# 111116/zdr

Measured on AMD Instinct MI355X. Metric: Msamples/s fwd+PRB-bwd, cbox 512x512 spp=256, higher is better.
Workload: dtype f32; 1 GPU; cbox path integrator 512x512 spp=256, forward + PRB backward w.r.t. the 1024x1024x4 material (BASELINE configs[2]); sampler=cmj, accel=brute, rccl_ranks=1, backend=none

## Files before the change

include/zdr.h:

```cpp
#ifndef ZDR_H
#define ZDR_H
#include <stdint.h>

#ifdef __cplusplus
extern "C" {
#endif

#define ZDR_VERSION_STRING "zdr-mi355x 0.3 (gfx950)"
#define ZDR_ABI_VERSION 4

enum { ZDR_OK = 0, ZDR_E_INVALID = -1, ZDR_E_HIP = -2, ZDR_E_UNSUPPORTED = -3, ZDR_E_NOMEM = -4 };

enum { ZDR_COLLOCATED = 0, ZDR_DIRECT = 1, ZDR_PATH = 2, ZDR_UVGRAD = 3 };
enum { ZDR_SAMPLER_CMJ = 0, ZDR_SAMPLER_PMJ02BN = 1 };
enum { ZDR_ACCEL_AUTO = 0, ZDR_ACCEL_BRUTE = 1, ZDR_ACCEL_BVH = 2 };
enum { ZDR_PRB_EXPECTATION = 0, ZDR_PRB_DETACHED = 1, ZDR_PRB_LITERAL = 2 };
#define ZDR_MAX_MATERIALS 16

typedef struct zdr_scene zdr_scene;

typedef struct {
    float fov;
    float origin[3], target[3], up[3];
} zdr_camera;
// ... 71 lines not shown
int zdr_render_stats(zdr_scene *scene, const zdr_render_params *params, const float *material,
                     uint64_t counters[8], void *stream);

int zdr_scene_check(zdr_scene *scene, void *stream);

int zdr_trace_closest(zdr_scene *scene, const float *rays, uint32_t n, int32_t *inst_prim, float *bary_t, void *stream);
int zdr_trace_any(zdr_scene *scene, const float *rays, uint32_t n, int32_t *occluded, void *stream);

int zdr_sampler_dump(zdr_scene *scene, int32_t sampler, uint32_t seed, uint32_t spp, const int32_t *queries,
                     uint32_t n, int32_t nvert, int32_t rr_depth, float *out, void *stream);

int zdr_vertex_sampler_dump(zdr_scene *scene, int32_t integrator, int32_t sampler, uint32_t seed, uint32_t spp,
                            const int32_t *queries, uint32_t n, int32_t nvert, int32_t rr_depth, float *out,
                            int32_t *batched, void *stream);

int zdr_path_dump(zdr_scene *scene, const zdr_render_params *params, const float *material, const float *d_image,
                  const int32_t *queries, uint32_t n, int32_t maxv, float *out, void *stream);

int zdr_debug_build_accel(const float *tri_xyz, uint32_t ntris, int accel, float *nodes_out, uint32_t nodes_cap,
                          uint32_t *nnodes, uint32_t *stack_entries, int32_t *order_out, float *isect_out);

int zdr_debug_never_occluders(const float *tri_xyz, uint32_t ntris, const uint8_t *is_light_tri, uint8_t *never_out);

#ifdef __cplusplus
}
#endif
#endif
```

zdr_amd/_native.py:

```python
from __future__ import annotations

import ctypes as C
import os

HERE = os.path.dirname(os.path.abspath(__file__))
LIB_PATH = os.path.join(HERE, "csrc", "libzdr_hip.so")

COLLOCATED, DIRECT, PATH, UVGRAD = 0, 1, 2, 3
SAMPLER_CMJ, SAMPLER_PMJ02BN = 0, 1
ACCEL_AUTO, ACCEL_BRUTE, ACCEL_BVH = 0, 1, 2
ABI_VERSION = 4
MAX_MATERIALS = 16
PRB_MODES = {"expectation": 0, "detached": 1, "literal": 2}
INTEGRATORS = {"collocated": COLLOCATED, "direct": DIRECT, "path": PATH}
SAMPLERS = {"cmj": SAMPLER_CMJ, "corrmj": SAMPLER_CMJ, "pmj02bn": SAMPLER_PMJ02BN}
ACCELS = {"auto": ACCEL_AUTO, "brute": ACCEL_BRUTE, "bvh": ACCEL_BVH}
COUNTER_NAMES = ("samples", "closest_rays", "closest_hits", "shadow_rays", "shaded_vertices",
                 "emitter_hits_bsdf", "nan_samples", "shadow_rays_traced")

EXPORTS = ("zdr_version", "zdr_abi_version", "zdr_last_error", "zdr_scene_create", "zdr_scene_destroy", "zdr_scene_info",
           "zdr_scene_set_emissions", "zdr_scene_set_envmap", "zdr_scene_set_pmj02bn_tables", "zdr_render_forward", "zdr_render_backward",
           "zdr_render_stats", "zdr_scene_check", "zdr_trace_closest", "zdr_trace_any", "zdr_sampler_dump", "zdr_vertex_sampler_dump", "zdr_path_dump", "zdr_debug_build_accel", "zdr_debug_never_occluders",
           "zdr_scene_set_material_slots", "zdr_render_forward_materials", "zdr_render_backward_materials",
           "zdr_scene_set_envmap_texture", "zdr_render_backward_env", "zdr_render_backward_materials_env",
           "zdr_scene_set_emission_values", "zdr_render_backward_emission", "zdr_render_backward_materials_emission")


class CameraPOD(C.Structure):
    _fields_ = [("fov", C.c_float), ("origin", C.c_float * 3), ("target", C.c_float * 3), ("up", C.c_float * 3)]


class RenderParams(C.Structure):
    _fields_ = [
        ("struct_size", C.c_uint32), ("integrator", C.c_int32), ("sampler", C.c_int32), ("width", C.c_int32), ("height", C.c_int32),
        ("spp", C.c_uint32), ("seed", C.c_uint32), ("use_tent", C.c_int32),
        ("x0", C.c_int32), ("y0", C.c_int32), ("x1", C.c_int32), ("y1", C.c_int32),
        ("sample_begin", C.c_uint32), ("sample_end", C.c_uint32),
        ("max_depth", C.c_int32), ("rr_depth", C.c_int32),
        ("camera", CameraPOD), ("tex_h", C.c_int32), ("tex_w", C.c_int32),
        ("tile_shard_index", C.c_int32), ("tile_shard_count", C.c_int32), ("prb_mode", C.c_int32),
    ]


class SceneInfo(C.Structure):
    _fields_ = [("ntris", C.c_uint32), ("nverts", C.c_uint32), ("ninst", C.c_uint32), ("light_count", C.c_uint32),
# ... 27 lines not shown
    L.zdr_scene_set_emissions.argtypes = [vp, fp, vp]
    L.zdr_scene_set_envmap.argtypes = [vp, fp, C.c_uint32, C.c_uint32, fp, ip, fp, C.c_uint32, C.c_uint32]
    L.zdr_scene_set_pmj02bn_tables.argtypes = [vp, vp, C.c_uint32, C.c_uint32, vp, C.c_uint32, C.c_uint32]
    L.zdr_render_forward.argtypes = [vp, C.POINTER(RenderParams), fp, fp, vp]
    L.zdr_render_backward.argtypes = [vp, C.POINTER(RenderParams), fp, fp, fp, vp]
    L.zdr_scene_set_material_slots.argtypes = [vp, ip, vp]
    L.zdr_render_forward_materials.argtypes = [vp, C.POINTER(RenderParams), fp, ip, C.c_uint32, fp, vp]
    L.zdr_render_backward_materials.argtypes = [vp, C.POINTER(RenderParams), fp, fp, ip, C.c_uint32, fp, vp]
    L.zdr_scene_set_envmap_texture.argtypes = [vp, fp, vp]
    L.zdr_render_backward_env.argtypes = [vp, C.POINTER(RenderParams), fp, fp, fp, fp, vp]
    L.zdr_render_backward_materials_env.argtypes = [vp, C.POINTER(RenderParams), fp, fp, ip, C.c_uint32, fp, fp, vp]
    L.zdr_scene_set_emission_values.argtypes = [vp, fp, vp]
    L.zdr_render_backward_emission.argtypes = [vp, C.POINTER(RenderParams), fp, fp, fp, fp, vp]
    L.zdr_render_backward_materials_emission.argtypes = [vp, C.POINTER(RenderParams), fp, fp, ip, C.c_uint32, fp, fp, vp]
    L.zdr_render_stats.argtypes = [vp, C.POINTER(RenderParams), fp, C.POINTER(C.c_uint64), vp]
    L.zdr_scene_check.argtypes = [vp, vp]
    L.zdr_trace_closest.argtypes = [vp, fp, C.c_uint32, ip, fp, vp]
    L.zdr_trace_any.argtypes = [vp, fp, C.c_uint32, ip, vp]
    L.zdr_sampler_dump.argtypes = [vp, C.c_int32, C.c_uint32, C.c_uint32, ip, C.c_uint32, C.c_int32, C.c_int32, fp, vp]
    L.zdr_vertex_sampler_dump.argtypes = [vp, C.c_int32, C.c_int32, C.c_uint32, C.c_uint32, ip, C.c_uint32, C.c_int32, C.c_int32, fp, C.POINTER(C.c_int32), vp]
    L.zdr_path_dump.argtypes = [vp, C.POINTER(RenderParams), fp, fp, ip, C.c_uint32, C.c_int32, fp, vp]
    L.zdr_debug_build_accel.argtypes = [fp, C.c_uint32, C.c_int, fp, C.c_uint32, C.POINTER(C.c_uint32), C.POINTER(C.c_uint32), ip, fp]
    L.zdr_debug_never_occluders.argtypes = [fp, C.c_uint32, vp, vp]
    for name in EXPORTS:
        getattr(L, name)
    if L.zdr_abi_version() != ABI_VERSION:
        raise ZdrError(f"{LIB_PATH} speaks ABI {L.zdr_abi_version()}, this binding ABI {ABI_VERSION}: rebuild (python -m zdr_amd.build --force)")
    _LIB = L
    return L


def check(rc: int):
    if rc != 0:
        raise ZdrError(f"libzdr_hip error {rc}: {lib().zdr_last_error().decode()}")
```

zdr_amd/csrc/accel.h:

```cpp
#pragma once
#include "scene.h"

#ifndef ZDR_MIN_WAVES
#define ZDR_MIN_WAVES 4
#endif
#ifndef ZDR_MIN_WAVES_ENV
#define ZDR_MIN_WAVES_ENV 4
#endif
#ifndef ZDR_MIN_WAVES_BVH
#define ZDR_MIN_WAVES_BVH 5
#endif
#ifndef ZDR_MIN_WAVES_BWD
#define ZDR_MIN_WAVES_BWD 4
#endif
#ifndef ZDR_POOL_SLOTS
#define ZDR_POOL_SLOTS 103
#endif
#ifndef ZDR_POOL_SLOTS_BVH
#define ZDR_POOL_SLOTS_BVH 56
#endif
#ifndef ZDR_MIN_WAVES_BWD_BVH
#define ZDR_MIN_WAVES_BWD_BVH 4
#endif

// ... 2 lines not shown
typedef const v4f __attribute__((address_space(4))) *const_v4f_ptr;
ZD const_v4f_ptr as_constant(const float4 *p) { return (const_v4f_ptr)(uintptr_t)p; }
ZD float4 f4(v4f a) { return make_float4(a.x, a.y, a.z, a.w); }

ZD bool tri_test(float4 N, float4 U, float4 V, f3 o, f3 d, float tmin, float tmax, float &t) {
    float nd = fmaf(N.z, d.z, fmaf(N.y, d.y, N.x * d.x));
    float no = fmaf(N.z, o.z, fmaf(N.y, o.y, N.x * o.x));
    float tt = (N.w - no) * rcp(nd);
    float px = fmaf(d.x, tt, o.x), py = fmaf(d.y, tt, o.y), pz = fmaf(d.z, tt, o.z);
    float uu = fmaf(U.z, pz, fmaf(U.y, py, U.x * px)) + U.w;
    float vv = fmaf(V.z, pz, fmaf(V.y, py, V.x * px)) + V.w;
    float c = fminf(fminf(uu, vv), 1.0f - (uu + vv));
    t = tt;
    return (tt > tmin) & (tt < tmax) & (c >= 0.0f);
}

ZD void hit_barycentrics(const DScene &S, Hit &h, f3 o, f3 d) {
    if (h.slot < 0) return;
    float4 U = S.isect[3 * (size_t)h.slot + 1], V = S.isect[3 * (size_t)h.slot + 2];
    f3 p = o + d * h.t;
    h.u = U.x * p.x + U.y * p.y + U.z * p.z + U.w;
    h.v = V.x * p.x + V.y * p.y + V.z * p.z + V.w;
}

typedef float v2f __attribute__((ext_vector_type(2)));
ZD v2f splat(float a) { v2f r = {a, a}; return r; }
ZD v2f pfma(v2f a, v2f b, v2f c) { return __builtin_elementwise_fma(a, b, c); }

struct PairHit { v2f t, c; };
ZD PairHit pair_test(const_v4f_ptr q, f3 o, f3 d) {
    v4f q0 = q[0], q1 = q[1];
    v2f dx = splat(d.x), dy = splat(d.y), dz = splat(d.z), ox = splat(o.x), oy = splat(o.y), oz = splat(o.z);
    v2f nd = pfma(q1.xy, dz, pfma(q0.zw, dy, q0.xy * dx));
    v2f no = pfma(q1.xy, oz, pfma(q0.zw, oy, q0.xy * ox));
    v2f tn = q1.zw - no;
    v2f r = {rcp(nd.x), rcp(nd.y)};
    PairHit h;
    h.t = tn * r;
    v2f px = pfma(dx, h.t, ox), py = pfma(dy, h.t, oy), pz = pfma(dz, h.t, oz);
    v2f e[4];
#pragma unroll
    for (int k = 0; k < 4; k++) {
        v4f a = q[2 + 2 * k], b = q[3 + 2 * k];
        e[k] = pfma(b.xy, pz, pfma(a.zw, py, a.xy * px)) + b.zw;
    }
    h.c.x = fminf(fminf(fminf(e[0].x, e[1].x), e[2].x), e[3].x);
    h.c.y = fminf(fminf(fminf(e[0].y, e[1].y), e[2].y), e[3].y);
    return h;
}

// ... 350 lines not shown
```

zdr_amd/csrc/integrators.h:

```cpp
#pragma once
#include <type_traits>
#include "accel.h"
#include "internal.h"
#include "microfacet.h"
#include "zdr.h"

ZD float tent_warp1(float u) {
    return (u < 0.5f) ? (fsqrt(2.0f * u) - 1.0f) : (1.0f - fsqrt(2.0f - 2.0f * u));
}

template <int SK, bool PACKED = false>
ZD void pixel_ray(const RenderCfg &R, const SamplerCfg &C, Sampler &smp, int x, int y, f3 &o, f3 &d) {
    f2 off = PACKED ? sampler_pixel_offset<SK>(C, smp) : sampler_next2<SK>(C, smp);
    if (R.use_tent) { off.x = tent_warp1(off.x) + 0.5f; off.y = tent_warp1(off.y) + 0.5f; }
    float px = R.two_over_w * ((float)x + off.x) - 1.0f;
    float py = R.two_over_h * ((float)y + off.y) - 1.0f;
    py *= R.aspect;
    px *= R.cam_tan; py *= R.cam_tan;
    o = ld3(R.cam_o);
    d = normalize((ld3(R.cam_right) * px - ld3(R.cam_upp) * py) + ld3(R.cam_fwd));
}

struct Counters { uint32_t c[8]; };
enum { C_SAMPLES, C_CLOSEST, C_HITS, C_SHADOW, C_SHADED, C_EMIT_BSDF, C_NAN, C_SHADOW_TRACED };
// ... 249 lines not shown
    else m = read_bsdf(io.material, it.uv, R.tex_h, R.tex_w);
    x.diffuse = mk3(m.x, m.y, m.z); x.roughness = m.w;
    COUNT(C_SHADED);
    if (BWD) {
        pv.uv = it.uv; pv.bW = mk3(0.0f); pv.cL = 0.0f; pv.dfLdr = 0.0f; pv.bpq = mk3(0.0f); pv.c = 0.0f; pv.dfdr = 0.0f;
        pv.T = mk3(0.0f); pv.fLW = mk3(0.0f); pv.bnorm = mk3(0.0f); pv.neeM = mk3(0.0f); pv.dlnp = 0.0f; pv.rr = 0;
    }
    x.onb = make_onb(it.ns);
    x.wo = to_local(x.onb, -ps.d);
    x.pre = (SK == 0) && !ENV && cmj_can_batch(C);
    x.u_lobe = 0.0f; x.u_dir.x = 0.0f; x.u_dir.y = 0.0f; x.i_rr = 0u;
    if (x.pre) {
        const VertexSamples v = cmj_vertex_samples(C, ps.smp);
        x.u_lobe = v.u_lobe; x.u_dir = v.u_dir; x.i_rr = v.i_rr;
        x.light = sample_light<ENV, LG>(S, it.p, v.u_pick, [&]() { return v.u_prim; }, [&]() { return v.u_pt; }, env_uv, mesh_light);
    } else {
        float u_pick = sampler_next<SK>(C, ps.smp);
        x.light = sample_light<ENV, LG>(S, it.p, u_pick, [&]() { return sampler_next<SK>(C, ps.smp); }, [&]() { return sampler_next2<SK>(C, ps.smp); }, env_uv, mesh_light);
    }
    x.wil = to_local(x.onb, x.light.wi);
    return x;
}

template <bool BWD, bool EG = false>
ZD NeeTerms nee_terms(const ShadeCtx &x, f3 beta_in, f3 *env_w = nullptr) {
    NeeTerms n; n.dL = n.bW = n.fLW = n.neeM = mk3(0.0f); n.cL = 0.0f; n.dfLdr = 0.0f;
    GgxTerms g = ggx_terms(x.wo, x.wil, x.roughness);
    f3 bsdf = ggx_brdf_from(g, x.wil, x.diffuse);
    float pb = ggx_pdf_from(g, x.wo, x.wil);
    float mis = balanced_heuristic(x.light.pdf, pb);
    float inv_dn = rcp(fmaxf(x.light.pdf, 1e-4f));
    n.dL = (((beta_in * bsdf) * mis) * x.light.eval) * inv_dn;
    if constexpr (EG) *env_w = ((beta_in * bsdf) * mis) * inv_dn;
    if (BWD) {
        f3 W = (x.light.eval * mis) * inv_dn;
        float dlnpL;
        n.bW = beta_in * W; n.cL = x.wil.z * ZDR_INV_PI; n.dfLdr = ggx_dfdr_from(g, x.wo, x.wil, x.roughness, dlnpL);
        n.fLW = bsdf * W;
        float pbf = (x.light.pdf + pb > 1e-4f) ? pb * rcp(x.light.pdf + pb) : 0.0f;
        n.neeM = ((beta_in * bsdf) * W) * (pbf * dlnpL);
    }
    return n;
}
template <bool BWD>
ZD void nee_apply(PathState &ps, PathVertex &pv, const NeeTerms &n) {
    ps.L = ps.L + n.dL;
    if (BWD) { pv.bW = n.bW; pv.cL = n.cL; pv.dfLdr = n.dfLdr; pv.fLW = n.fLW; pv.neeM = n.neeM; }
}

template <int SK, bool BWD>
ZD bool sample_bsdf(const RenderCfg &R, const SamplerCfg &C, const ShadeCtx &x, PathState &ps, const Interaction &it, PathVertex &pv) {
    float u_lobe = x.u_lobe; f2 u_dir = x.u_dir;
    if (!x.pre) { u_lobe = sampler_next<SK>(C, ps.smp); u_dir = sampler_next2<SK>(C, ps.smp); }
    f3 wi_local = ggx_sample(x.wo, x.roughness, u_lobe, u_dir);
    GgxTerms g = ggx_terms(x.wo, wi_local, x.roughness);
    ps.pdf_bsdf = ggx_pdf_from(g, x.wo, wi_local);
    f3 wi = to_world(x.onb, wi_local);
    bool stop = (dot(wi, it.ng) < 1e-4f) || (wi_local.z < 1e-4f);
    const f3 beta_in = ps.beta;
    float q = 1.0f;
    int rr_kind = 0;
    if (!stop) {
        ps.o = offset_ray_origin(it.p, it.ng); ps.d = wi;
        f3 f = ggx_brdf_from(g, wi_local, x.diffuse);
        float inv_p = rcp(ps.pdf_bsdf);
        ps.beta = ps.beta * (f * inv_p);
        if (ps.depth >= R.rr_depth) {
            float l = 0.212671f * ps.beta.x + 0.715160f * ps.beta.y + 0.072169f * ps.beta.z;
            if (l == 0.0f) stop = true;
            else {
                q = fmaxf(l, 0.05f);
                float r = x.pre ? cmj_next_with_index(C, ps.smp, x.i_rr) : sampler_next<SK>(C, ps.smp);
                if (r >= q) stop = true;
                else { ps.beta = ps.beta * rcp(q); rr_kind = (l >= 1.0f) ? 2 : ((l >= 0.05f) ? 1 : 0); }
            }
        }
        if (BWD && !stop) {
            float inv_pq = inv_p * rcp(q);
            pv.bpq = beta_in * inv_pq; pv.c = wi_local.z * ZDR_INV_PI; pv.dfdr = ggx_dfdr_from(g, x.wo, wi_local, x.roughness, pv.dlnp);
            pv.T = f * inv_pq;
            pv.rr = rr_kind;
            if (rr_kind == 2) pv.bnorm = ps.beta;
            if (R.prb_mode == ZDR_PRB_LITERAL) pv.bnorm = beta_in * (f * inv_p);
        }
    }
    ps.depth++;
    if (ps.depth >= R.max_depth) stop = true;
    return stop;
}

struct VertexRays { bool shadow, stop; f3 sd; float stmax; };
template <int SK, bool BWD, bool STATS, bool ENV, bool MT = false, bool EG = false, bool LG = false>
ZD VertexRays path_vertex_begin(const DScene &S, const RenderCfg &R, const SamplerCfg &C, const KernelIO &io,
                                PathState &ps, const Interaction &it, PathVertex &pv, NeeTerms &n, Counters &cnt, EnvTerm *env = nullptr, EmitTerm *emit = nullptr) {
    f2 env_uv; env_uv.x = -1.0f; env_uv.y = 0.0f;
    int mesh_light = -1;
    const ShadeCtx x = shade_ctx<SK, BWD, STATS, ENV, MT, LG>(S, R, C, io, ps, it, pv, cnt, EG ? &env_uv : nullptr, LG ? &mesh_light : nullptr);
    VertexRays vr; vr.sd = x.light.wi; vr.stmax = x.light.dist;
    n.dL = n.bW = n.fLW = n.neeM = mk3(0.0f); n.cL = 0.0f; n.dfLdr = 0.0f;
    if constexpr (EG) env_term_clear(*env);
    if constexpr (LG) emit_term_clear(*emit);
    COUNT(C_SHADOW);
    vr.shadow = x.wil.z >= 1e-4f;
    if (vr.shadow) {
        if constexpr (LG) {
            n = nee_terms<BWD, true>(x, ps.beta, &emit->w);
            emit->light = mesh_light;
        } else
        if constexpr (EG) {
            n = nee_terms<BWD, true>(x, ps.beta, &env->w);
            if (env_uv.x < 0.0f) env->w = mk3(0.0f);
            env->uv = env_uv;
        } else n = nee_terms<BWD>(x, ps.beta);
        bool nothing = (n.dL.x == 0.0f) & (n.dL.y == 0.0f) & (n.dL.z == 0.0f) &&
                       (!BWD || ((n.bW.x == 0.0f) & (n.bW.y == 0.0f) & (n.bW.z == 0.0f) & (n.fLW.x == 0.0f) & (n.fLW.y == 0.0f) & (n.fLW.z == 0.0f) &
                                 (n.neeM.x == 0.0f) & (n.neeM.y == 0.0f) & (n.neeM.z == 0.0f) & (fabsf(n.dfLdr) < 3.0e38f)));
        if constexpr (EG) nothing = nothing && (env->w.x == 0.0f) & (env->w.y == 0.0f) & (env->w.z == 0.0f);
        vr.shadow = !nothing;
    }
    if (vr.shadow) COUNT(C_SHADOW_TRACED);
    vr.stop = sample_bsdf<SK, BWD>(R, C, x, ps, it, pv);
    if (!vr.stop) COUNT(C_CLOSEST);
    return vr;
}

template <int SK, class A, bool BWD, bool STATS, bool ENV, bool MT = false, bool EG = false, bool LG = false>
ZD bool path_shade(const DScene &S, const RenderCfg &R, const SamplerCfg &C, const KernelIO &io, int *lds,
                   PathState &ps, const Interaction &it, PathVertex &pv, Hit &h, Counters &cnt, EnvTerm *env = nullptr, EmitTerm *emit = nullptr) {
    static_assert(!LG || (BWD && !EG), "the emission gradient is a backward mode of its own");
    if constexpr (A::kFuseRays) {
        NeeTerms n;
        const VertexRays vr = path_vertex_begin<SK, BWD, STATS, ENV, MT, EG, LG>(S, R, C, io, ps, it, pv, n, cnt, env, emit);
        bool occluded;
        A::shadow_and_closest(S, lds, vr.shadow, it.p, vr.sd, 1e-4f, vr.stmax, !vr.stop, ps.o, ps.d, occluded, h);
        if (vr.shadow && !occluded) nee_apply<BWD>(ps, pv, n);
        else if constexpr (EG) env->w = mk3(0.0f);
        else if constexpr (LG) emit->light = -1;
        return vr.stop;
    } else if constexpr (LG) {
        int mesh_light = -1;
        const ShadeCtx x = shade_ctx<SK, BWD, STATS, ENV, MT, true>(S, R, C, io, ps, it, pv, cnt, nullptr, &mesh_light);
        const bool occluded = A::any_shadow(S, lds, it.p, x.light.wi, 1e-4f, x.light.dist);
        emit_term_clear(*emit);
        if (!occluded && x.wil.z >= 1e-4f) {
            nee_apply<BWD>(ps, pv, nee_terms<BWD, true>(x, ps.beta, &emit->w));
            emit->light = mesh_light;
        }
        return sample_bsdf<SK, BWD>(R, C, x, ps, it, pv);
    } else if constexpr (EG) {
        f2 env_uv; env_uv.x = -1.0f; env_uv.y = 0.0f;
        const ShadeCtx x = shade_ctx<SK, BWD, STATS, ENV, MT>(S, R, C, io, ps, it, pv, cnt, &env_uv);
        const bool occluded = A::any_shadow(S, lds, it.p, x.light.wi, 1e-4f, x.light.dist);
        env_term_clear(*env);
        if (!occluded && x.wil.z >= 1e-4f) {
            nee_apply<BWD>(ps, pv, nee_terms<BWD, true>(x, ps.beta, &env->w));
            if (env_uv.x < 0.0f) env->w = mk3(0.0f);
            env->uv = env_uv;
        }
        return sample_bsdf<SK, BWD>(R, C, x, ps, it, pv);
    } else {
        const ShadeCtx x = shade_ctx<SK, BWD, STATS, ENV, MT>(S, R, C, io, ps, it, pv, cnt);
        COUNT(C_SHADOW);
        const bool occluded = A::any_shadow(S, lds, it.p, x.light.wi, 1e-4f, x.light.dist);
        if (!occluded && x.wil.z >= 1e-4f) nee_apply<BWD>(ps, pv, nee_terms<BWD>(x, ps.beta));
        COUNT(C_SHADOW_TRACED);
        return sample_bsdf<SK, BWD>(R, C, x, ps, it, pv);
    }
}

template <class A, bool STATS>
ZD void path_continue(const DScene &S, int *lds, const PathState &ps, Hit &h, Counters &cnt) {
    if constexpr (!A::kFuseRays) { COUNT(C_CLOSEST); h = A::closest(S, lds, ps.o, ps.d, 0.0f, 1e30f); }
}

struct PrimaryQueue { float4 *base; uint32_t head, tail; };
#define ZDR_QUEUE_ENTRIES (ZDR_RING_CAP * 64)
static_assert(ZDR_RING_BATCH * 64 + 64 <= ZDR_QUEUE_ENTRIES, "a refill must fit behind a queue that could not serve every idle lane");

ZD PrimaryQueue queue_init(const KernelIO &io) {
    PrimaryQueue r; r.base = io.ring + (size_t)blockIdx.x * (ZDR_QUEUE_ENTRIES * 2); r.head = 0; r.tail = 0;
    return r;
}
ZD uint32_t lane_rank(unsigned long long mask) {
    return __builtin_amdgcn_mbcnt_hi((unsigned)(mask >> 32), __builtin_amdgcn_mbcnt_lo((unsigned)mask, 0u));
}

struct NoEnvMiss { ZD void operator()(const EnvTerm &) const {} };
struct NoEmitHit { ZD void operator()(const EmitTerm &) const {} };
template <int SK, class A, bool BWD, bool STATS, bool ENV, bool MT = false, class MISS = NoEnvMiss, class EMIT = NoEmitHit>
ZD void primary_refill(const DScene &S, const RenderCfg &R, const SamplerCfg &C, int *lds, int x, int y, bool valid, unsigned long long cam_mask,
// ... 114 lines not shown
```

zdr_amd/csrc/internal.h:

```cpp
#pragma once
#include <hip/hip_runtime.h>
#include <stdint.h>
#include "sampler.h"
#include "scene.h"
#include "zdr.h"

#define ZDR_MAX_RECORDED_DEPTH 16

#ifndef ZDR_RING_CAP
#define ZDR_RING_CAP 16
#endif
#ifndef ZDR_RING_BATCH
#define ZDR_RING_BATCH 8
#endif

#define ZDR_MAX_PERSISTENT_BLOCKS 8192

struct MaterialSlot { int32_t texel, h, w, cell, copies, stride; };
#define ZDR_ENV_CELL_BUDGET (1u << 22)
static_assert(ZDR_ENV_ENTRY == ZDR_MAX_MATERIALS - 1, "the environment-gradient calls keep the map in the last entry of the material table");
struct MaterialTable {
    const int32_t *inst_slot;
    int32_t nmat, ncells;
    MaterialSlot m[ZDR_MAX_MATERIALS];
// ... 30 lines not shown
    float *cells;
    unsigned long long *counters;
    const unsigned long long *tile_masks;
    int32_t tile_masks_valid;
    unsigned int *work_counters;
    float4 *ring;
    MaterialTable mt;
};

struct RenderLaunch {
    int integrator, accel_is_bvh, backward, stats;
    float *d_env;
    float *d_emission;
};
int zdr_launch_render(const DScene &S, const RenderCfg &R, const SamplerCfg &C, const KernelIO &io, const RenderLaunch &L, hipStream_t stream);
#define ZDR_EMISSION_COPIES 256
int zdr_launch_set_emission_values(const DScene &S, const float *src, float *emission, float4 *emission4, float4 *light_tris, hipStream_t stream);
int zdr_launch_zero(void *p, size_t bytes, hipStream_t stream);
int zdr_launch_copy(void *dst, const void *src, size_t bytes, hipStream_t stream);
int zdr_launch_trace(const DScene &S, int accel_is_bvh, int any, const float *rays, uint32_t n,
                     int32_t *out_i, float *out_f, hipStream_t stream);
int zdr_launch_sampler_dump(const SamplerCfg &C, const int32_t *queries, uint32_t n, int32_t nvert,
                            int32_t rr_depth, float *out, int as_path_kernels, int *batched, hipStream_t stream);
int zdr_launch_path_dump(const DScene &S, const RenderCfg &R, const SamplerCfg &C, const KernelIO &io, int accel_is_bvh,
                         const int32_t *queries, uint32_t n, int32_t maxv, float *out, hipStream_t stream);
```

zdr_amd/csrc/microfacet.h:

```cpp
#pragma once
#include "vecmath.h"

#define ZDR_SPECULAR 0.04f

ZD float pow5(float x) { float x2 = x * x; return x2 * x2 * x; }

struct GgxTerms {
    float a2;
    float D, F, G1i, G1o;
    float t;
    float nh2;
    float ki, ko;
    float si, so;
    float inv4;
    float wo_dot_h;
};

ZD GgxTerms ggx_terms(f3 wo, f3 wi, float roughness) {
    GgxTerms g;
    float alpha = roughness * roughness;
    g.a2 = alpha * alpha;
    f3 h = normalize(wi + wo);
    float nh = fmaxf(0.00001f, h.z);
    g.nh2 = nh * nh;
// ... 18 lines not shown
    return (mk3(s) + diffuse * ZDR_INV_PI) * wi.z;
}

ZD float ggx_pdf_from(const GgxTerms &g, f3 wo, f3 wi) {
    float a = fabsf(g.wo_dot_h);
    float pdf_wm = g.G1o * rcp(fabsf(wo.z)) * g.D * a;
    float glossy = pdf_wm * rcp(4.0f * a);
    return 0.5f * (wi.z * ZDR_INV_PI) + 0.5f * glossy;
}

ZD float ggx_dfdr_from(const GgxTerms &g, f3 wo, f3 wi, float roughness, float &dlnpdf_dr) {
    float t3 = g.t * g.t * g.t;
    float dD = (1.0f - g.nh2 * (1.0f + g.a2)) * rcp(ZDR_PI * t3);
    float opi = 1.0f + g.si, opo = 1.0f + g.so;
    float dG1i = -g.ki * rcp(g.si * (opi * opi));
    float dG1o = -g.ko * rcp(g.so * (opo * opo));
    float dS = dD * (g.G1i * g.G1o) + g.D * (dG1i * g.G1o + g.G1i * dG1o);
    float r3 = roughness * roughness * roughness;
    float dglossy = (dG1o * g.D + g.G1o * dD) * rcp(4.0f * fabsf(wo.z));
    dlnpdf_dr = (0.5f * dglossy * 4.0f * r3) * rcp(ggx_pdf_from(g, wo, wi));
    return 4.0f * r3 * (g.F * wi.z * g.inv4) * dS;
}

ZD f3 sample_wm_disk(f3 w, float alpha, float px, float py) {
    f3 wh = normalize(mk3(alpha * w.x, alpha * w.y, w.z));
    if (wh.z < 0.0f) wh = -wh;
    f3 T1 = (wh.z < 0.99999f) ? normalize(cross(mk3(0.0f, 0.0f, 1.0f), wh)) : mk3(1.0f, 0.0f, 0.0f);
    f3 T2 = cross(wh, T1);
    float h = fsqrt(1.0f - px * px);
    py = lerpf(h, py, (1.0f + wh.z) * 0.5f);
    float pz = fsqrt(fmaxf(0.0f, 1.0f - (px * px + py * py)));
    f3 nh = px * T1 + py * T2 + pz * wh;
    return normalize(mk3(alpha * nh.x, alpha * nh.y, fmaxf(1e-6f, nh.z)));
}

ZD f3 ggx_sample(f3 wo, float roughness, float u_lobe, f2 u2) {
    float r = fsqrt(u2.x), phi = 2.0f * ZDR_PI * u2.y;
    float sn, cs;
    sincosf(phi, &sn, &cs);
    float px = r * cs, py = r * sn;
    if (u_lobe < 0.5f) return mk3(px, py, fsqrt(1.0f - u2.x));
    f3 wm = sample_wm_disk(wo, roughness * roughness, px, py);
    f3 i = -wo;
    return i - wm * (2.0f * dot(wm, i));
}
```

zdr_amd/csrc/vecmath.h:

```cpp
#pragma once
#include <hip/hip_runtime.h>
#include <stdint.h>

#define ZD __device__ __forceinline__

struct f3 { float x, y, z; };
struct f2 { float x, y; };

ZD f3 mk3(float x, float y, float z) { f3 r; r.x = x; r.y = y; r.z = z; return r; }
ZD f3 mk3(float s) { return mk3(s, s, s); }
ZD f3 operator+(f3 a, f3 b) { return mk3(a.x + b.x, a.y + b.y, a.z + b.z); }
ZD f3 operator-(f3 a, f3 b) { return mk3(a.x - b.x, a.y - b.y, a.z - b.z); }
ZD f3 operator*(f3 a, f3 b) { return mk3(a.x * b.x, a.y * b.y, a.z * b.z); }
ZD f3 operator*(f3 a, float s) { return mk3(a.x * s, a.y * s, a.z * s); }
ZD f3 operator*(float s, f3 a) { return mk3(a.x * s, a.y * s, a.z * s); }
ZD f3 operator-(f3 a) { return mk3(-a.x, -a.y, -a.z); }
ZD float dot(f3 a, f3 b) { return a.x * b.x + a.y * b.y + a.z * b.z; }
ZD f3 cross(f3 a, f3 b) { return mk3(a.y * b.z - a.z * b.y, a.z * b.x - a.x * b.z, a.x * b.y - a.y * b.x); }

ZD float rcp(float x) { return __builtin_amdgcn_rcpf(x); }
ZD float rsq(float x) { return __builtin_amdgcn_rsqf(x); }
ZD float fsqrt(float x) { return __builtin_amdgcn_sqrtf(x); }
ZD f3 operator/(f3 a, float s) { float r = rcp(s); return mk3(a.x * r, a.y * r, a.z * r); }
ZD f3 normalize(f3 a) { return a * rsq(dot(a, a)); }
ZD float length(f3 a) { return fsqrt(dot(a, a)); }
ZD bool any_nan(f3 a) { return (a.x != a.x) | (a.y != a.y) | (a.z != a.z); }
ZD float clampf(float x, float lo, float hi) { return fminf(fmaxf(x, lo), hi); }
ZD int clampi(int x, int lo, int hi) { return min(max(x, lo), hi); }
ZD float lerpf(float a, float b, float t) { return a + t * (b - a); }
ZD f3 ld3(const float *p) { return mk3(p[0], p[1], p[2]); }

#define ZDR_PI 3.14159265358979323846f
#define ZDR_INV_PI 0.31830988618379067154f
```

zdr_amd/csrc/zdr_api.cpp:

```cpp
#include <algorithm>
#include <cmath>
#include <cstdlib>
#include <cstring>
#include <map>
#include <string>
#include <vector>

#include "internal.h"
#include "zdr.h"

static thread_local std::string g_err;
static int fail(int code, const std::string &msg) { g_err = msg; return code; }
#define HIPCHK(expr) do { hipError_t e_ = (expr); if (e_ != hipSuccess) return fail(ZDR_E_HIP, std::string(#expr) + ": " + hipGetErrorString(e_)); } while (0)

extern "C" const char *zdr_version(void) { return ZDR_VERSION_STRING; }
extern "C" int zdr_abi_version(void) { return ZDR_ABI_VERSION; }
extern "C" const char *zdr_last_error(void) { return g_err.c_str(); }

struct h3 { float x, y, z; };
static inline h3 H3(float x, float y, float z) { return {x, y, z}; }
static inline h3 hsub(h3 a, h3 b) { return {a.x - b.x, a.y - b.y, a.z - b.z}; }
static inline h3 hcross(h3 a, h3 b) { return {a.y * b.z - a.z * b.y, a.z * b.x - a.x * b.z, a.x * b.y - a.y * b.x}; }
static inline float hdot(h3 a, h3 b) { return a.x * b.x + a.y * b.y + a.z * b.z; }
static inline h3 hscale(h3 a, float s) { return {a.x * s, a.y * s, a.z * s}; }
// ... 1214 lines not shown
    if (maxv < 1 || maxv > ZDR_MAX_RECORDED_DEPTH) return fail(ZDR_E_INVALID, "maxv must lie in [1, 16]");
    HIPCHK(hipSetDevice(s->device));
    RenderCfg R; SamplerCfg C;
    int rc = make_render_cfg(p, true, R); if (rc) return rc;
    rc = make_sampler_cfg(s, p->sampler, p->seed, p->spp, C); if (rc) return rc;
    KernelIO io; memset(&io, 0, sizeof io);
    io.material = (const float4 *)material; io.d_image = (const float4 *)d_image;
    DScene S = s->ds;
    S.shadow_pairs = (S.env_count > 0) ? ~0ull : s->shadow_pairs;
    if (zdr_launch_path_dump(S, R, C, io, s->accel_is_bvh, queries, n, maxv, out, (hipStream_t)stream)) return fail(ZDR_E_HIP, "path dump launch failed");
    return ZDR_OK;
}

extern "C" int zdr_sampler_dump(zdr_scene *s, int32_t sampler, uint32_t seed, uint32_t spp, const int32_t *queries, uint32_t n,
                                int32_t nvert, int32_t rr_depth, float *out, void *stream) {
    if (!s || !queries || !out || nvert < 0) return fail(ZDR_E_INVALID, "bad argument");
    HIPCHK(hipSetDevice(s->device));
    SamplerCfg C;
    int rc = make_sampler_cfg(s, sampler, seed, spp, C); if (rc) return rc;
    if (zdr_launch_sampler_dump(C, queries, n, nvert, rr_depth, out, 0, nullptr, (hipStream_t)stream)) return fail(ZDR_E_HIP, "sampler dump launch failed");
    return ZDR_OK;
}

extern "C" int zdr_vertex_sampler_dump(zdr_scene *s, int32_t integrator, int32_t sampler, uint32_t seed, uint32_t spp, const int32_t *queries, uint32_t n,
                                       int32_t nvert, int32_t rr_depth, float *out, int32_t *batched, void *stream) {
    if (!s || !queries || !out || nvert < 0) return fail(ZDR_E_INVALID, "bad argument");
    if (integrator != ZDR_PATH && integrator != ZDR_DIRECT) return fail(ZDR_E_INVALID, "the path and the direct integrator have draw routes of their own");
    HIPCHK(hipSetDevice(s->device));
    SamplerCfg C;
    int rc = make_sampler_cfg(s, sampler, seed, spp, C); if (rc) return rc;
    int b = 0;
    if (zdr_launch_sampler_dump(C, queries, n, nvert, rr_depth, out, integrator == ZDR_DIRECT ? 2 : 1, &b, (hipStream_t)stream)) return fail(ZDR_E_HIP, "sampler dump launch failed");
    if (batched) *batched = b;
    return ZDR_OK;
}
```

zdr_amd/csrc/zdr_kernels.hip:

```cpp
#include <algorithm>
#include <cstddef>
#include <cstdlib>
#include <map>
#include <mutex>
#include <tuple>
#include <type_traits>
#include "integrators.h"
#include "zdr.h"

#define WAVE 64

struct WorkItem { int x, y, pix; bool valid; uint32_t s_begin, s_end; int chunk, tile, tile_local; };

ZD WorkItem decode_item(const RenderCfg &R, int logical) {
    const int nblocks = R.ntiles * R.nchunks;
    WorkItem w;
    w.valid = logical >= 0 && logical < nblocks;
    const int tl = w.valid ? logical / R.nchunks : 0;
    w.chunk = w.valid ? logical - tl * R.nchunks : 0;
    const int number = tl * R.shard_count + R.shard_index;
    const int ty = number / R.tiles_x;
    int tx = number - ty * R.tiles_x + ty * R.shard_skew;
    tx -= (tx / R.tiles_x) * R.tiles_x;
    w.tile = ty * R.tiles_x + tx; w.tile_local = tl;
// ... 1009 lines not shown
    if (!any_nan(ps.L) && nv > 0) {
        SweepState sw; sw.A = le_grad * term_Li; sw.Lv = sw.A; sw.s = 0.0f; sw.Z = 0.0f; sw.tw = (R.prb_mode != ZDR_PRB_EXPECTATION) ? 0.0f : plfrac * dot(ps.beta, sw.A);
        for (int k = nv - 1; k >= 0; k--) {
            f2 guv; const float4 g = sweep_vertex(recs[k], sw, guv, R.prb_mode);
            if (k < maxv) { float *q = o + 8 + 24 * k; q[12] = g.x; q[13] = g.y; q[14] = g.z; q[15] = g.w; }
        }
    }
}

int zdr_launch_path_dump(const DScene &S_in, const RenderCfg &R, const SamplerCfg &C, const KernelIO &io, int accel_is_bvh,
                         const int32_t *queries, uint32_t n, int32_t maxv, float *out, hipStream_t st) {
    DScene S = S_in;
    if (n == 0) return 0;
    dim3 grid((n + WAVE - 1) / WAVE);
    const size_t dyn = accel_is_bvh ? bvh_dyn_lds(S, true, true) : 0;
    with_sampler_accel(C.kind, accel_is_bvh, [&](auto sk, auto acc) {
        with_bool(S.env_count > 0, [&](auto env) {
            hipLaunchKernelGGL((k_path_dump<decltype(sk)::value, typename decltype(acc)::type, decltype(env)::value>), grid, dim3(WAVE), dyn, st, S, R, C, io, queries, n, maxv, out);
        });
    });
    return hipGetLastError() == hipSuccess ? 0 : -1;
}

template <int SK>
__global__ void k_sampler_dump(SamplerCfg C, const int32_t *q, uint32_t n, int nvert, int rr_depth, float *out) {
    uint32_t i = blockIdx.x * blockDim.x + threadIdx.x;
    if (i >= n) return;
    uint32_t px = (uint32_t)q[3 * i], py = (uint32_t)q[3 * i + 1], idx = (uint32_t)q[3 * i + 2];
    uint32_t perm_seed = (SK == 0) ? xxhash32_4(px, py, C.seed, 0u) : 0u;
    Sampler s = sampler_make<SK>(C, px, py, perm_seed, idx);
    const int stride = 2 + 8 * nvert;
    float *o = out + (size_t)i * stride;
    int k = 0;
    f2 u = sampler_next2<SK>(C, s); o[k++] = u.x; o[k++] = u.y;
    for (int v = 0; v < nvert; v++) {
        o[k++] = sampler_next<SK>(C, s); o[k++] = sampler_next<SK>(C, s);
        u = sampler_next2<SK>(C, s); o[k++] = u.x; o[k++] = u.y;
        o[k++] = sampler_next<SK>(C, s);
        u = sampler_next2<SK>(C, s); o[k++] = u.x; o[k++] = u.y;
        if (v >= rr_depth) o[k++] = sampler_next<SK>(C, s);
    }
    for (; k < stride; k++) o[k] = 0.0f;
}

template <int SK>
__global__ void k_vertex_sampler_dump(SamplerCfg C, const int32_t *q, uint32_t n, int nvert, int rr_depth, int direct, float *out) {
// ... 45 lines not shown
```

Baseline: 7606 Msamples/s.

## Evaluate NEE and sampled-direction GGX BRDFs together as packed pairs

Restructures path vertex shading so the BSDF direction is sampled up front and the GGX terms for both the light direction and the sampled direction are computed in one paired evaluation using two-wide float vectors. This targets packed FMA use and shares the outgoing-direction terms between the two evaluations. It also unifies the non-fused accelerator path: in backward mode the shadow ray is traced before shading instead of after. A debug kernel comparing paired and scalar evaluation is added. The price is that BSDF terms are now computed for the light direction even when the NEE sample is later discarded, and register pressure may rise.

Result: no change. 7655 Msamples/s, median of 6 (+0.6%).

```diff
diff --git a/include/zdr.h b/include/zdr.h
--- a/include/zdr.h
+++ b/include/zdr.h
@@ -117,6 +117,8 @@
 
 int zdr_debug_never_occluders(const float *tri_xyz, uint32_t ntris, const uint8_t *is_light_tri, uint8_t *never_out);
 
+int zdr_debug_brdf_pair(const float *in, uint32_t n, float *out, void *stream);
+
 #ifdef __cplusplus
 }
 #endif
diff --git a/zdr_amd/_native.py b/zdr_amd/_native.py
--- a/zdr_amd/_native.py
+++ b/zdr_amd/_native.py
@@ -20,7 +20,7 @@
 
 EXPORTS = ("zdr_version", "zdr_abi_version", "zdr_last_error", "zdr_scene_create", "zdr_scene_destroy", "zdr_scene_info",
            "zdr_scene_set_emissions", "zdr_scene_set_envmap", "zdr_scene_set_pmj02bn_tables", "zdr_render_forward", "zdr_render_backward",
-           "zdr_render_stats", "zdr_scene_check", "zdr_trace_closest", "zdr_trace_any", "zdr_sampler_dump", "zdr_vertex_sampler_dump", "zdr_path_dump", "zdr_debug_build_accel", "zdr_debug_never_occluders",
+           "zdr_render_stats", "zdr_scene_check", "zdr_trace_closest", "zdr_trace_any", "zdr_sampler_dump", "zdr_vertex_sampler_dump", "zdr_path_dump", "zdr_debug_build_accel", "zdr_debug_never_occluders", "zdr_debug_brdf_pair",
            "zdr_scene_set_material_slots", "zdr_render_forward_materials", "zdr_render_backward_materials",
            "zdr_scene_set_envmap_texture", "zdr_render_backward_env", "zdr_render_backward_materials_env",
            "zdr_scene_set_emission_values", "zdr_render_backward_emission", "zdr_render_backward_materials_emission")
@@ -94,6 +94,7 @@
     L.zdr_path_dump.argtypes = [vp, C.POINTER(RenderParams), fp, fp, ip, C.c_uint32, C.c_int32, fp, vp]
     L.zdr_debug_build_accel.argtypes = [fp, C.c_uint32, C.c_int, fp, C.c_uint32, C.POINTER(C.c_uint32), C.POINTER(C.c_uint32), ip, fp]
     L.zdr_debug_never_occluders.argtypes = [fp, C.c_uint32, vp, vp]
+    L.zdr_debug_brdf_pair.argtypes = [fp, C.c_uint32, fp, vp]
     for name in EXPORTS:
         getattr(L, name)
     if L.zdr_abi_version() != ABI_VERSION:
diff --git a/zdr_amd/csrc/accel.h b/zdr_amd/csrc/accel.h
--- a/zdr_amd/csrc/accel.h
+++ b/zdr_amd/csrc/accel.h
@@ -48,10 +48,6 @@
     h.u = U.x * p.x + U.y * p.y + U.z * p.z + U.w;
     h.v = V.x * p.x + V.y * p.y + V.z * p.z + V.w;
 }
-
-typedef float v2f __attribute__((ext_vector_type(2)));
-ZD v2f splat(float a) { v2f r = {a, a}; return r; }
-ZD v2f pfma(v2f a, v2f b, v2f c) { return __builtin_elementwise_fma(a, b, c); }
 
 struct PairHit { v2f t, c; };
 ZD PairHit pair_test(const_v4f_ptr q, f3 o, f3 d) {
diff --git a/zdr_amd/csrc/integrators.h b/zdr_amd/csrc/integrators.h
--- a/zdr_amd/csrc/integrators.h
+++ b/zdr_amd/csrc/integrators.h
@@ -295,23 +295,36 @@
     return x;
 }
 
+struct BsdfEval { f3 f; float pdf, dfdr, dlnp; };
+template <bool BWD>
+ZD void bsdf_eval_pair(const ShadeCtx &x, f3 wi_local, BsdfEval &l, BsdfEval &s) {
+    const GgxPair g = ggx_pair(x.wo, x.wil, wi_local, x.roughness);
+    ggx_brdf_pair(g, x.diffuse, l.f, s.f);
+    const v2f pdf = ggx_pdf_pair(g);
+    l.pdf = pdf.x; s.pdf = pdf.y;
+    l.dfdr = s.dfdr = l.dlnp = s.dlnp = 0.0f;
+    if (BWD) {
+        v2f dlnp;
+        const v2f dfdr = ggx_dfdr_pair(g, x.wo, x.roughness, pdf, dlnp);
+        l.dfdr = dfdr.x; s.dfdr = dfdr.y; l.dlnp = dlnp.x; s.dlnp = dlnp.y;
+    }
+}
+
 template <bool BWD, bool EG = false>
-ZD NeeTerms nee_terms(const ShadeCtx &x, f3 beta_in, f3 *env_w = nullptr) {
+ZD NeeTerms nee_terms(const ShadeCtx &x, const BsdfEval &e, f3 beta_in, f3 *env_w = nullptr) {
     NeeTerms n; n.dL = n.bW = n.fLW = n.neeM = mk3(0.0f); n.cL = 0.0f; n.dfLdr = 0.0f;
-    GgxTerms g = ggx_terms(x.wo, x.wil, x.roughness);
-    f3 bsdf = ggx_brdf_from(g, x.wil, x.diffuse);
-    float pb = ggx_pdf_from(g, x.wo, x.wil);
+    const f3 bsdf = e.f;
+    const float pb = e.pdf;
     float mis = balanced_heuristic(x.light.pdf, pb);
     float inv_dn = rcp(fmaxf(x.light.pdf, 1e-4f));
     n.dL = (((beta_in * bsdf) * mis) * x.light.eval) * inv_dn;
     if constexpr (EG) *env_w = ((beta_in * bsdf) * mis) * inv_dn;
     if (BWD) {
         f3 W = (x.light.eval * mis) * inv_dn;
-        float dlnpL;
-        n.bW = beta_in * W; n.cL = x.wil.z * ZDR_INV_PI; n.dfLdr = ggx_dfdr_from(g, x.wo, x.wil, x.roughness, dlnpL);
+        n.bW = beta_in * W; n.cL = x.wil.z * ZDR_INV_PI; n.dfLdr = e.dfdr;
         n.fLW = bsdf * W;
         float pbf = (x.light.pdf + pb > 1e-4f) ? pb * rcp(x.light.pdf + pb) : 0.0f;
-        n.neeM = ((beta_in * bsdf) * W) * (pbf * dlnpL);
+        n.neeM = ((beta_in * bsdf) * W) * (pbf * e.dlnp);
     }
     return n;
 }
@@ -321,13 +334,16 @@
     if (BWD) { pv.bW = n.bW; pv.cL = n.cL; pv.dfLdr = n.dfLdr; pv.fLW = n.fLW; pv.neeM = n.neeM; }
 }
 
-template <int SK, bool BWD>
-ZD bool sample_bsdf(const RenderCfg &R, const SamplerCfg &C, const ShadeCtx &x, PathState &ps, const Interaction &it, PathVertex &pv) {
+template <int SK>
+ZD f3 sample_dir(const SamplerCfg &C, const ShadeCtx &x, PathState &ps) {
     float u_lobe = x.u_lobe; f2 u_dir = x.u_dir;
     if (!x.pre) { u_lobe = sampler_next<SK>(C, ps.smp); u_dir = sampler_next2<SK>(C, ps.smp); }
-    f3 wi_local = ggx_sample(x.wo, x.roughness, u_lobe, u_dir);
-    GgxTerms g = ggx_terms(x.wo, wi_local, x.roughness);
-    ps.pdf_bsdf = ggx_pdf_from(g, x.wo, wi_local);
+    return ggx_sample(x.wo, x.roughness, u_lobe, u_dir);
+}
+
+template <int SK, bool BWD>
+ZD bool sample_bsdf(const RenderCfg &R, const SamplerCfg &C, const ShadeCtx &x, f3 wi_local, const BsdfEval &e, PathState &ps, const Interaction &it, PathVertex &pv) {
+    ps.pdf_bsdf = e.pdf;
     f3 wi = to_world(x.onb, wi_local);
     bool stop = (dot(wi, it.ng) < 1e-4f) || (wi_local.z < 1e-4f);
     const f3 beta_in = ps.beta;
@@ -335,7 +351,7 @@
     int rr_kind = 0;
     if (!stop) {
         ps.o = offset_ray_origin(it.p, it.ng); ps.d = wi;
-        f3 f = ggx_brdf_from(g, wi_local, x.diffuse);
+        f3 f = e.f;
         float inv_p = rcp(ps.pdf_bsdf);
         ps.beta = ps.beta * (f * inv_p);
         if (ps.depth >= R.rr_depth) {
@@ -350,7 +366,7 @@
         }
         if (BWD && !stop) {
             float inv_pq = inv_p * rcp(q);
-            pv.bpq = beta_in * inv_pq; pv.c = wi_local.z * ZDR_INV_PI; pv.dfdr = ggx_dfdr_from(g, x.wo, wi_local, x.roughness, pv.dlnp);
+            pv.bpq = beta_in * inv_pq; pv.c = wi_local.z * ZDR_INV_PI; pv.dfdr = e.dfdr; pv.dlnp = e.dlnp;
             pv.T = f * inv_pq;
             pv.rr = rr_kind;
             if (rr_kind == 2) pv.bnorm = ps.beta;
@@ -362,38 +378,45 @@
     return stop;
 }
 
-struct VertexRays { bool shadow, stop; f3 sd; float stmax; };
-template <int SK, bool BWD, bool STATS, bool ENV, bool MT = false, bool EG = false, bool LG = false>
-ZD VertexRays path_vertex_begin(const DScene &S, const RenderCfg &R, const SamplerCfg &C, const KernelIO &io,
+struct VertexRays { bool shadow, stop, occluded; f3 sd; float stmax; };
+template <int SK, class A, bool BWD, bool STATS, bool ENV, bool MT = false, bool EG = false, bool LG = false>
+ZD VertexRays path_vertex_begin(const DScene &S, const RenderCfg &R, const SamplerCfg &C, const KernelIO &io, int *lds,
                                 PathState &ps, const Interaction &it, PathVertex &pv, NeeTerms &n, Counters &cnt, EnvTerm *env = nullptr, EmitTerm *emit = nullptr) {
     f2 env_uv; env_uv.x = -1.0f; env_uv.y = 0.0f;
     int mesh_light = -1;
+    constexpr bool FUSED = A::kFuseRays, TRACE_FIRST = !A::kFuseRays && BWD;
     const ShadeCtx x = shade_ctx<SK, BWD, STATS, ENV, MT, LG>(S, R, C, io, ps, it, pv, cnt, EG ? &env_uv : nullptr, LG ? &mesh_light : nullptr);
-    VertexRays vr; vr.sd = x.light.wi; vr.stmax = x.light.dist;
+    VertexRays vr; vr.sd = x.light.wi; vr.stmax = x.light.dist; vr.occluded = false;
+    if constexpr (TRACE_FIRST) vr.occluded = A::any_shadow(S, lds, it.p, vr.sd, 1e-4f, vr.stmax);
+    const f3 wi_local = sample_dir<SK>(C, x, ps);
+    BsdfEval el, es;
+    bsdf_eval_pair<BWD>(x, wi_local, el, es);
     n.dL = n.bW = n.fLW = n.neeM = mk3(0.0f); n.cL = 0.0f; n.dfLdr = 0.0f;
     if constexpr (EG) env_term_clear(*env);
     if constexpr (LG) emit_term_clear(*emit);
     COUNT(C_SHADOW);
-    vr.shadow = x.wil.z >= 1e-4f;
+    vr.shadow = (x.wil.z >= 1e-4f) && !vr.occluded;
     if (vr.shadow) {
         if constexpr (LG) {
-            n = nee_terms<BWD, true>(x, ps.beta, &emit->w);
+            n = nee_terms<BWD, true>(x, el, ps.beta, &emit->w);
             emit->light = mesh_light;
         } else
         if constexpr (EG) {
-            n = nee_terms<BWD, true>(x, ps.beta, &env->w);
+            n = nee_terms<BWD, true>(x, el, ps.beta, &env->w);
             if (env_uv.x < 0.0f) env->w = mk3(0.0f);
             env->uv = env_uv;
-        } else n = nee_terms<BWD>(x, ps.beta);
-        bool nothing = (n.dL.x == 0.0f) & (n.dL.y == 0.0f) & (n.dL.z == 0.0f) &&
-                       (!BWD || ((n.bW.x == 0.0f) & (n.bW.y == 0.0f) & (n.bW.z == 0.0f) & (n.fLW.x == 0.0f) & (n.fLW.y == 0.0f) & (n.fLW.z == 0.0f) &
-                                 (n.neeM.x == 0.0f) & (n.neeM.y == 0.0f) & (n.neeM.z == 0.0f) & (fabsf(n.dfLdr) < 3.0e38f)));
-        if constexpr (EG) nothing = nothing && (env->w.x == 0.0f) & (env->w.y == 0.0f) & (env->w.z == 0.0f);
-        vr.shadow = !nothing;
-    }
-    if (vr.shadow) COUNT(C_SHADOW_TRACED);
-    vr.stop = sample_bsdf<SK, BWD>(R, C, x, ps, it, pv);
-    if (!vr.stop) COUNT(C_CLOSEST);
+        } else n = nee_terms<BWD>(x, el, ps.beta);
+        if constexpr (FUSED) {
+            bool nothing = (n.dL.x == 0.0f) & (n.dL.y == 0.0f) & (n.dL.z == 0.0f) &&
+                           (!BWD || ((n.bW.x == 0.0f) & (n.bW.y == 0.0f) & (n.bW.z == 0.0f) & (n.fLW.x == 0.0f) & (n.fLW.y == 0.0f) & (n.fLW.z == 0.0f) &
+                                     (n.neeM.x == 0.0f) & (n.neeM.y == 0.0f) & (n.neeM.z == 0.0f) & (fabsf(n.dfLdr) < 3.0e38f)));
+            if constexpr (EG) nothing = nothing && (env->w.x == 0.0f) & (env->w.y == 0.0f) & (env->w.z == 0.0f);
+            vr.shadow = !nothing;
+        }
+    }
+    if (vr.shadow || !FUSED) COUNT(C_SHADOW_TRACED);
+    vr.stop = sample_bsdf<SK, BWD>(R, C, x, wi_local, es, ps, it, pv);
+    if (FUSED && !vr.stop) COUNT(C_CLOSEST);
     return vr;
 }
 
@@ -401,44 +424,15 @@
 ZD bool path_shade(const DScene &S, const RenderCfg &R, const SamplerCfg &C, const KernelIO &io, int *lds,
                    PathState &ps, const Interaction &it, PathVertex &pv, Hit &h, Counters &cnt, EnvTerm *env = nullptr, EmitTerm *emit = nullptr) {
     static_assert(!LG || (BWD && !EG), "the emission gradient is a backward mode of its own");
-    if constexpr (A::kFuseRays) {
-        NeeTerms n;
-        const VertexRays vr = path_vertex_begin<SK, BWD, STATS, ENV, MT, EG, LG>(S, R, C, io, ps, it, pv, n, cnt, env, emit);
-        bool occluded;
-        A::shadow_and_closest(S, lds, vr.shadow, it.p, vr.sd, 1e-4f, vr.stmax, !vr.stop, ps.o, ps.d, occluded, h);
-        if (vr.shadow && !occluded) nee_apply<BWD>(ps, pv, n);
-        else if constexpr (EG) env->w = mk3(0.0f);
-        else if constexpr (LG) emit->light = -1;
-        return vr.stop;
-    } else if constexpr (LG) {
-        int mesh_light = -1;
-        const ShadeCtx x = shade_ctx<SK, BWD, STATS, ENV, MT, true>(S, R, C, io, ps, it, pv, cnt, nullptr, &mesh_light);
-        const bool occluded = A::any_shadow(S, lds, it.p, x.light.wi, 1e-4f, x.light.dist);
-        emit_term_clear(*emit);
-        if (!occluded && x.wil.z >= 1e-4f) {
-            nee_apply<BWD>(ps, pv, nee_terms<BWD, true>(x, ps.beta, &emit->w));
-            emit->light = mesh_light;
-        }
-        return sample_bsdf<SK, BWD>(R, C, x, ps, it, pv);
-    } else if constexpr (EG) {
-        f2 env_uv; env_uv.x = -1.0f; env_uv.y = 0.0f;
-        const ShadeCtx x = shade_ctx<SK, BWD, STATS, ENV, MT>(S, R, C, io, ps, it, pv, cnt, &env_uv);
-        const bool occluded = A::any_shadow(S, lds, it.p, x.light.wi, 1e-4f, x.light.dist);
-        env_term_clear(*env);
-        if (!occluded && x.wil.z >= 1e-4f) {
-            nee_apply<BWD>(ps, pv, nee_terms<BWD, true>(x, ps.beta, &env->w));
-            if (env_uv.x < 0.0f) env->w = mk3(0.0f);
-            env->uv = env_uv;
-        }
-        return sample_bsdf<SK, BWD>(R, C, x, ps, it, pv);
-    } else {
-        const ShadeCtx x = shade_ctx<SK, BWD, STATS, ENV, MT>(S, R, C, io, ps, it, pv, cnt);
-        COUNT(C_SHADOW);
-        const bool occluded = A::any_shadow(S, lds, it.p, x.light.wi, 1e-4f, x.light.dist);
-        if (!occluded && x.wil.z >= 1e-4f) nee_apply<BWD>(ps, pv, nee_terms<BWD>(x, ps.beta));
-        COUNT(C_SHADOW_TRACED);
-        return sample_bsdf<SK, BWD>(R, C, x, ps, it, pv);
-    }
+    NeeTerms n;
+    const VertexRays vr = path_vertex_begin<SK, A, BWD, STATS, ENV, MT, EG, LG>(S, R, C, io, lds, ps, it, pv, n, cnt, env, emit);
+    bool occluded = vr.occluded;
+    if constexpr (A::kFuseRays) A::shadow_and_closest(S, lds, vr.shadow, it.p, vr.sd, 1e-4f, vr.stmax, !vr.stop, ps.o, ps.d, occluded, h);
+    else if constexpr (!BWD) occluded = A::any_shadow(S, lds, it.p, vr.sd, 1e-4f, vr.stmax);
+    if (vr.shadow && !occluded) nee_apply<BWD>(ps, pv, n);
+    else if constexpr (EG) env->w = mk3(0.0f);
+    else if constexpr (LG) emit->light = -1;
+    return vr.stop;
 }
 
 template <class A, bool STATS>
diff --git a/zdr_amd/csrc/internal.h b/zdr_amd/csrc/internal.h
--- a/zdr_amd/csrc/internal.h
+++ b/zdr_amd/csrc/internal.h
@@ -76,5 +76,6 @@
                      int32_t *out_i, float *out_f, hipStream_t stream);
 int zdr_launch_sampler_dump(const SamplerCfg &C, const int32_t *queries, uint32_t n, int32_t nvert,
                             int32_t rr_depth, float *out, int as_path_kernels, int *batched, hipStream_t stream);
+int zdr_launch_brdf_pair(const float *in, uint32_t n, float *out, hipStream_t stream);
 int zdr_launch_path_dump(const DScene &S, const RenderCfg &R, const SamplerCfg &C, const KernelIO &io, int accel_is_bvh,
                          const int32_t *queries, uint32_t n, int32_t maxv, float *out, hipStream_t stream);
diff --git a/zdr_amd/csrc/microfacet.h b/zdr_amd/csrc/microfacet.h
--- a/zdr_amd/csrc/microfacet.h
+++ b/zdr_amd/csrc/microfacet.h
@@ -64,6 +64,69 @@
     return 4.0f * r3 * (g.F * wi.z * g.inv4) * dS;
 }
 
+struct GgxPair {
+    float a2, G1o, ko, so, inv_awoz;
+    v2f D, F, G1i, t, nh2, ki, si, inv4, wo_dot_h, wiz;
+};
+
+ZD GgxPair ggx_pair(f3 wo, f3 wiA, f3 wiB, float roughness) {
+    GgxPair g;
+    float alpha = roughness * roughness;
+    g.a2 = alpha * alpha;
+    float nvo = fmaxf(0.00001f, wo.z);
+    g.ko = (1.0f - nvo * nvo) * rcp(nvo * nvo);
+    g.so = fsqrt(1.0f + g.a2 * g.ko);
+    g.G1o = 2.0f * rcp(1.0f + g.so);
+    g.inv_awoz = rcp(fabsf(wo.z));
+    float ax = wiA.x, ay = wiA.y, az = wiA.z;
+    asm("" : "+v"(ax), "+v"(ay), "+v"(az));
+    g.wiz = mk2(az, wiB.z);
+    v2f sx = mk2(ax, wiB.x) + splat(wo.x), sy = mk2(ay, wiB.y) + splat(wo.y), sz = g.wiz + splat(wo.z);
+    v2f inv_len = prsq(sx * sx + sy * sy + sz * sz);
+    v2f hx = sx * inv_len, hy = sy * inv_len, hz = sz * inv_len;
+    v2f nh = pmaxs(0.00001f, hz);
+    g.nh2 = nh * nh;
+    g.t = g.nh2 * splat(g.a2 - 1.0f) + splat(1.0f);
+    g.D = splat(g.a2) * prcp(splat(ZDR_PI) * (g.t * g.t));
+    g.wo_dot_h = splat(wo.x) * hx + splat(wo.y) * hy + splat(wo.z) * hz;
+    v2f c = mk2(clampf(g.wo_dot_h.x, 0.00001f, 1.0f), clampf(g.wo_dot_h.y, 0.00001f, 1.0f));
+    v2f m = splat(1.0f) - c, m2 = m * m;
+    g.F = splat(ZDR_SPECULAR) + splat(1.0f - ZDR_SPECULAR) * (m2 * m2 * m);
+    v2f nvi = pmaxs(0.00001f, g.wiz);
+    g.ki = (splat(1.0f) - nvi * nvi) * prcp(nvi * nvi);
+    g.si = psqrt(splat(1.0f) + splat(g.a2) * g.ki);
+    g.G1i = splat(2.0f) * prcp(splat(1.0f) + g.si);
+    g.inv4 = prcp(splat(4.0f) * nvi * splat(nvo));
+    return g;
+}
+
+ZD void ggx_brdf_pair(const GgxPair &g, f3 diffuse, f3 &fA, f3 &fB) {
+    v2f s = (g.D * g.F * (g.G1i * splat(g.G1o))) * g.inv4;
+    const v2f ipi = splat(ZDR_INV_PI);
+    v2f r = pfma(splat(diffuse.x), ipi, s) * g.wiz, gr = pfma(splat(diffuse.y), ipi, s) * g.wiz, b = pfma(splat(diffuse.z), ipi, s) * g.wiz;
+    fA = mk3(r.x, gr.x, b.x); fB = mk3(r.y, gr.y, b.y);
+}
+
+ZD v2f ggx_pdf_pair(const GgxPair &g) {
+    v2f a = pabs(g.wo_dot_h);
+    v2f pdf_wm = splat(g.G1o * g.inv_awoz) * g.D * a;
+    v2f glossy = pdf_wm * prcp(splat(4.0f) * a);
+    return splat(0.5f) * (g.wiz * splat(ZDR_INV_PI)) + splat(0.5f) * glossy;
+}
+
+ZD v2f ggx_dfdr_pair(const GgxPair &g, f3 wo, float roughness, v2f pdf, v2f &dlnpdf_dr) {
+    v2f t3 = g.t * g.t * g.t;
+    v2f dD = (splat(1.0f) - g.nh2 * splat(1.0f + g.a2)) * prcp(splat(ZDR_PI) * t3);
+    v2f opi = splat(1.0f) + g.si; float opo = 1.0f + g.so;
+    v2f dG1i = -g.ki * prcp(g.si * (opi * opi));
+    float dG1o = -g.ko * rcp(g.so * (opo * opo));
+    v2f dS = dD * (g.G1i * splat(g.G1o)) + g.D * (dG1i * splat(g.G1o) + g.G1i * splat(dG1o));
+    float r3 = roughness * roughness * roughness;
+    v2f dglossy = (splat(dG1o) * g.D + splat(g.G1o) * dD) * splat(rcp(4.0f * fabsf(wo.z)));
+    dlnpdf_dr = (splat(0.5f) * dglossy * splat(4.0f) * splat(r3)) * prcp(pdf);
+    return splat(4.0f * r3) * (g.F * g.wiz * g.inv4) * dS;
+}
+
 ZD f3 sample_wm_disk(f3 w, float alpha, float px, float py) {
     f3 wh = normalize(mk3(alpha * w.x, alpha * w.y, w.z));
     if (wh.z < 0.0f) wh = -wh;
diff --git a/zdr_amd/csrc/vecmath.h b/zdr_amd/csrc/vecmath.h
--- a/zdr_amd/csrc/vecmath.h
+++ b/zdr_amd/csrc/vecmath.h
@@ -30,5 +30,15 @@
 ZD float lerpf(float a, float b, float t) { return a + t * (b - a); }
 ZD f3 ld3(const float *p) { return mk3(p[0], p[1], p[2]); }
 
+typedef float v2f __attribute__((ext_vector_type(2)));
+ZD v2f splat(float a) { v2f r = {a, a}; return r; }
+ZD v2f mk2(float a, float b) { v2f r = {a, b}; return r; }
+ZD v2f pfma(v2f a, v2f b, v2f c) { return __builtin_elementwise_fma(a, b, c); }
+ZD v2f prcp(v2f a) { return mk2(rcp(a.x), rcp(a.y)); }
+ZD v2f prsq(v2f a) { return mk2(rsq(a.x), rsq(a.y)); }
+ZD v2f psqrt(v2f a) { return mk2(fsqrt(a.x), fsqrt(a.y)); }
+ZD v2f pmaxs(float lo, v2f a) { return mk2(fmaxf(lo, a.x), fmaxf(lo, a.y)); }
+ZD v2f pabs(v2f a) { return mk2(fabsf(a.x), fabsf(a.y)); }
+
 #define ZDR_PI 3.14159265358979323846f
 #define ZDR_INV_PI 0.31830988618379067154f
diff --git a/zdr_amd/csrc/zdr_api.cpp b/zdr_amd/csrc/zdr_api.cpp
--- a/zdr_amd/csrc/zdr_api.cpp
+++ b/zdr_amd/csrc/zdr_api.cpp
@@ -1260,6 +1260,12 @@
     return ZDR_OK;
 }
 
+extern "C" int zdr_debug_brdf_pair(const float *in, uint32_t n, float *out, void *stream) {
+    if (!in || !out) return fail(ZDR_E_INVALID, "bad argument");
+    if (zdr_launch_brdf_pair(in, n, out, (hipStream_t)stream)) return fail(ZDR_E_HIP, "brdf pair launch failed");
+    return ZDR_OK;
+}
+
 extern "C" int zdr_vertex_sampler_dump(zdr_scene *s, int32_t integrator, int32_t sampler, uint32_t seed, uint32_t spp, const int32_t *queries, uint32_t n,
                                        int32_t nvert, int32_t rr_depth, float *out, int32_t *batched, void *stream) {
     if (!s || !queries || !out || nvert < 0) return fail(ZDR_E_INVALID, "bad argument");
diff --git a/zdr_amd/csrc/zdr_kernels.hip b/zdr_amd/csrc/zdr_kernels.hip
--- a/zdr_amd/csrc/zdr_kernels.hip
+++ b/zdr_amd/csrc/zdr_kernels.hip
@@ -1055,6 +1055,39 @@
     return hipGetLastError() == hipSuccess ? 0 : -1;
 }
 
+template <bool PAIR>
+__global__ void k_brdf_pair(const float *__restrict__ in, uint32_t n, float *__restrict__ out) {
+    uint32_t i = blockIdx.x * blockDim.x + threadIdx.x;
+    if (i >= n) return;
+    const float *q = in + (size_t)i * 13;
+    const f3 wo = ld3(q), wiA = ld3(q + 3), wiB = ld3(q + 6), diffuse = ld3(q + 10);
+    const float roughness = q[9];
+    float *o = out + (size_t)i * 24 + (PAIR ? 12 : 0);
+    f3 fA, fB; v2f pdf, dfdr, dlnp;
+    if constexpr (PAIR) {
+        const GgxPair p = ggx_pair(wo, wiA, wiB, roughness);
+        ggx_brdf_pair(p, diffuse, fA, fB);
+        pdf = ggx_pdf_pair(p);
+        dfdr = ggx_dfdr_pair(p, wo, roughness, pdf, dlnp);
+    } else {
+        const GgxTerms a = ggx_terms(wo, wiA, roughness), b = ggx_terms(wo, wiB, roughness);
+        fA = ggx_brdf_from(a, wiA, diffuse); fB = ggx_brdf_from(b, wiB, diffuse);
+        pdf = mk2(ggx_pdf_from(a, wo, wiA), ggx_pdf_from(b, wo, wiB));
+        float la, lb;
+        dfdr = mk2(ggx_dfdr_from(a, wo, wiA, roughness, la), ggx_dfdr_from(b, wo, wiB, roughness, lb));
+        dlnp = mk2(la, lb);
+    }
+    o[0] = fA.x; o[1] = fA.y; o[2] = fA.z; o[3] = pdf.x; o[4] = dfdr.x; o[5] = dlnp.x;
+    o[6] = fB.x; o[7] = fB.y; o[8] = fB.z; o[9] = pdf.y; o[10] = dfdr.y; o[11] = dlnp.y;
+}
+
+int zdr_launch_brdf_pair(const float *in, uint32_t n, float *out, hipStream_t st) {
+    if (n == 0) return 0;
+    hipLaunchKernelGGL(k_brdf_pair<false>, dim3((n + 63) / 64), dim3(64), 0, st, in, n, out);
+    hipLaunchKernelGGL(k_brdf_pair<true>, dim3((n + 63) / 64), dim3(64), 0, st, in, n, out);
+    return hipGetLastError() == hipSuccess ? 0 : -1;
+}
+
 template <int SK>
 __global__ void k_sampler_dump(SamplerCfg C, const int32_t *q, uint32_t n, int nvert, int rr_depth, float *out) {
     uint32_t i = blockIdx.x * blockDim.x + threadIdx.x;
```
